# leonsick/s2d

Measured on AMD Instinct MI355X. Metric: clip-frames/sec fwd+loss, R50 M2F-Video T=8 720p Q=100, higher is better.
Workload: dtype f32 (f16x3 MFMA for dense contractions); 1 GPU; KDVideoMaskFormer fwd+loss (student+teacher fwd, GT+KD VideoSetCriterion), c4: 2 clips/GPU x T=8 x 720x1280, Q=100, P=160000, N=10 sparse GT instances/clip, encoder dropout 0.3; clips_per_gpu=2, frames_per_clip=8, parallelism=dp1 (clips sharded, no collective), streams=2

## Files before the change

include/s2d_hip.h:

```cpp
#ifndef S2D_HIP_H
#define S2D_HIP_H
#include <stdint.h>

#ifndef HIP_INCLUDE_HIP_HIP_RUNTIME_API_H
typedef struct ihipStream_t *hipStream_t;
#endif

#ifdef __cplusplus
extern "C" {
#endif

#define S2D_OK 0
#define S2D_ERR_ARG (-1)
#define S2D_ERR_LAUNCH (-2)

int s2d_abi_version(void);

int s2d_set_dense_mode(int mode);


int s2d_gemm_nt_f32(const float *A, const float *B, float *C, int M, int N, int K, long lda, long ldb, long ldc,
                    int batch, long strideA, long strideB, long strideC, const float *scale, const float *bias,
                    const float *res, long ldr, long strideR, int res_rows, int res_cols, int relu, const void *B_split,
                    hipStream_t stream);

int s2d_gemm_nt_dropout_f32(const float *A, const float *B, float *C, int M, int N, int K, long lda, long ldb, long ldc,
                            const float *bias, const float *res, long ldr, int relu, const void *B_split, float p,
                            uint64_t seed, unsigned site, unsigned row0, hipStream_t stream);

int s2d_dropout_f32(const float *x, long M, int N, float p, uint64_t seed, unsigned site, unsigned row0, float *y, hipStream_t stream);

int s2d_gemm_nt_gate_f32(const float *A, const float *B, float *C, int M, int N, int K, long lda, long ldb, long ldc, const float *scale,
                         const float *res, long ldr, const float *gate, long ldg, float gate_scale, const void *B_split, hipStream_t stream);
int s2d_conv2d_nhwc_gate_f32(const float *x, const float *w, float *y, int N, int H, int W, int Cin, int Cout, int KH, int KW, int stride,
                             int pad, const float *scale, const float *gate, float gate_scale, const void *w_split, hipStream_t stream);
int s2d_gemm_nt_presplit_f32(const void *A_split, const float *B, float *C, int M, int N, int K, long ldb, long ldc, const float *bias,
                             const float *res, long ldr, int res_rows, int res_cols, int relu, const void *B_split, hipStream_t stream);
long s2d_split_weights_words(int N, int K);
int s2d_split_weights_f16(const float *W, int N, int K, long ldw, void *out, hipStream_t stream);

long s2d_ffn_pack_words(int C, int F, int Npost, int pre);
int s2d_ffn_pack_f16(const float *W1, const float *W2, int C, int F, const float *Wpost, int Npost, const float *Wpre, void *out,
                     hipStream_t stream);
int s2d_ffn_fused_f32(const float *x, long M, int C, int F, const void *pack, const float *b1, const float *b2, const float *ln1_gamma,
                      const float *ln1_beta, const float *ln2_gamma, const float *ln2_beta, float eps, float p, uint64_t seed,
                      unsigned site_hidden, unsigned site_out, unsigned row0, float *xn, float *y, int Npost, const float *post_bias,
                      const float *post_pos, int post_S, int post_npos, long post_ldpos, float *post_out, long post_ld,
                      const float *pre_bias, const float *pre_res, unsigned site_pre, hipStream_t stream);

int s2d_conv2d_nhwc_f32(const float *x, const float *w, float *y, int N, int H, int W, int Cin, int Cout, int KH,
                        int KW, int stride, int pad, const float *scale, const float *bias, const float *res,
                        int relu, const void *w_split, hipStream_t stream);

int s2d_gemm_nt_amp_f32(const float *A, const float *B, float *C, int M, int N, int K, long lda, long ldb, long ldc, int batch,
                        long strideA, long strideB, long strideC, const float *scale, const float *bias, const float *res, long ldr,
                        long strideR, int res_rows, int res_cols, int relu, hipStream_t stream);
int s2d_conv2d_nhwc_amp_f32(const float *x, const float *w, float *y, int N, int H, int W, int Cin, int Cout, int KH, int KW, int stride,
                            int pad, const float *scale, const float *bias, const float *res, int relu, hipStream_t stream);


int s2d_msda_forward_f32(const float *value, const int64_t *shapes_host, const int64_t *level_start_host,
                         const float *loc, const float *attn_w, int N, int S, int M, int D, int L, int Lq, int P,
                         float *out, hipStream_t stream);

int s2d_msda_backward_f32(const float *value, const int64_t *shapes_host, const int64_t *level_start_host,
                          const float *loc, const float *attn_w, const float *grad_out, int N, int S, int M, int D,
                          int L, int Lq, int P, float *grad_value, float *grad_loc, float *grad_attn_w,
                          hipStream_t stream);

long s2d_msda_backward_workspace_bytes(const int64_t *shapes_host, int N, int M, int L, int Lq, int P);
int s2d_msda_backward_sorted_f32(const float *value, const int64_t *shapes_host, const int64_t *level_start_host,
                                 const float *loc, const float *attn_w, const float *grad_out, int N, int S, int M, int D,
                                 int L, int Lq, int P, float *grad_value, float *grad_loc, float *grad_attn_w, void *workspace,
                                 long workspace_bytes, hipStream_t stream);
int s2d_msda_backward_sorted_strided_f32(const float *value, long ldv, const int64_t *shapes_host, const int64_t *level_start_host,
                                         const float *loc, const float *attn_w, const float *grad_out, int N, int S, int M, int D,
                                         int L, int Lq, int P, float *grad_value, long ldg, float *grad_loc, float *grad_attn_w,
                                         void *workspace, long workspace_bytes, hipStream_t stream);

long s2d_msda_dev_forward_workspace_bytes(void);
int s2d_msda_forward_dev_f32(const float *value, const int64_t *shapes_dev, const int64_t *level_start_dev, const float *loc,
                             const float *attn_w, int N, int S, int M, int D, int L, int Lq, int P, float *out, void *workspace,
                             hipStream_t stream);
long s2d_msda_dev_backward_workspace_bytes(int N, int S, int M, int L, int Lq, int P);
int s2d_msda_backward_dev_f32(const float *value, const int64_t *shapes_dev, const int64_t *level_start_dev, const float *loc,
                              const float *attn_w, const float *grad_out, int N, int S, int M, int D, int L, int Lq, int P,
                              float *grad_value, float *grad_loc, float *grad_attn_w, void *workspace, long workspace_bytes,
                              hipStream_t stream);
int s2d_msda_forward_dev_f64(const double *value, const int64_t *shapes_dev, const int64_t *level_start_dev, const double *loc,
                             const double *attn_w, int N, int S, int M, int D, int L, int Lq, int P, double *out, hipStream_t stream);
int s2d_msda_backward_dev_f64(const double *value, const int64_t *shapes_dev, const int64_t *level_start_dev, const double *loc,
                              const double *attn_w, const double *grad_out, int N, int S, int M, int D, int L, int Lq, int P,
                              double *grad_value, double *grad_loc, double *grad_attn_w, hipStream_t stream);

int s2d_msda_dev_error_word(int *word);
int s2d_msda_dev_status(const void *workspace, int *err_host, hipStream_t stream);

int s2d_msda_fused_forward_f32(const float *value, int ldv, const int64_t *shapes_host, const float *offs_logits, int ldoa,
                               int N, int S, int M, int D, int L, int P, float *out, hipStream_t stream);

int s2d_msda_fused_prep_f32(const float *offs_logits, int ldoa, const int64_t *shapes_host, int N, int S, int M, int L, int P,
                            float *loc, float *attn, hipStream_t stream);
int s2d_msda_fused_chain_f32(const float *attn, const float *grad_loc, const float *grad_attn, const int64_t *shapes_host, int N,
                             int S, int M, int L, int P, float *d_offs_logits, int ldd, hipStream_t stream);
int s2d_msda_fused_backward_query_f32(const float *value, int ldv, const int64_t *shapes_host, const float *offs_logits, int ldoa,
                                      const float *grad_out, int N, int S, int M, int D, int L, int P, float *d_offs_logits, int ldd,
                                      hipStream_t stream);


int s2d_normalize_pad_nhwc4_f32(const uint8_t *frames, int F, int H0, int W0, int Hp, int Wp, const float *mean3_host,
                                const float *std3_host, float *out, hipStream_t stream);

int s2d_maxpool3x3s2_nhwc_f32(const float *x, int N, int H, int W, int C, float *y, hipStream_t stream);
int s2d_maxpool3x3s2_nhwc_idx_f32(const float *x, int N, int H, int W, int C, float *y, unsigned char *argmax, hipStream_t stream);

long s2d_groupnorm_workspace_doubles(int N, int H, int W, int G);
int s2d_groupnorm_nhwc_f32(const float *x, int N, int H, int W, int C, int G, const float *gamma, const float *beta,
                           float eps, const float *up, int hu, int wu, int relu, double *stats_ws, float *y,
                           hipStream_t stream);

int s2d_layernorm_f32(const float *x, const float *res, const float *gamma, const float *beta, long rows, int C,
                      float eps, float *y, hipStream_t stream);

int s2d_add_bcast_f32(const float *x, const float *b, long n, long bn, float *y, hipStream_t stream);

int s2d_pe_sine_f32(int T, int H, int W, int num_pos_feats, const float *add_c, float *out, hipStream_t stream);


int s2d_attn_mask_bits(const float *mask_logits, int ldq, int B, int Q, int T, int hm, int wm, int hl, int wl, int compact,
                       uint32_t *bits, uint32_t *unmasked, hipStream_t stream);

long s2d_attn_workspace_floats(int B, int H, int K);

int s2d_masked_attn_f32(const float *q, const float *k, const float *v, long ldk, long ldv, const uint32_t *bits,
                        const uint32_t *unmasked, int B, int Q, int K, int C, int H, float *workspace, float *out, float *lse,
                        hipStream_t stream);

long s2d_attn_backward_workspace_floats(int B, int H, int K);
int s2d_masked_attn_backward_f32(const float *q, const float *k, const float *v, long ldk, long ldv, const uint32_t *bits,
                                 const uint32_t *unmasked, const float *out, const float *lse, const float *dout, int B, int Q,
                                 int K, int C, int H, float *workspace, float *dq, float *dk, float *dv, hipStream_t stream);
int s2d_masked_attn_backward_strided_f32(const float *q, const float *k, const float *v, long ldk, long ldv, const uint32_t *bits,
                                         const uint32_t *unmasked, const float *out, const float *lse, const float *dout, int B, int Q,
                                         int K, int C, int H, float *workspace, float *dq, float *dk, long lddk, float *dv, long lddv,
                                         hipStream_t stream);


long s2d_matcher_workspace_floats(int NL, int B, int T, int P, int H, int W);

int s2d_matcher_cost_f32(const float *mask_logits, const float *class_logits, const uint8_t *tgt, const int *tgt_count,
                         const float *coords, uint64_t seed, int NL, int B, int Q, int ldq, int T, int hm, int wm, int H,
                         int W, int Nmax, int P, float w_class, float w_mask, float w_dice, float *workspace, float *C,
                         hipStream_t stream);

long s2d_matcher_c_workspace_floats(int NL, int B, int Q, int T, int P, int H, int W);
int s2d_matcher_cost_c_f32(const float *mask_logits, const float *class_logits, int C1, const uint8_t *tgt, const int *tgt_count,
                           const float *coords, uint64_t seed, int NL, int B, int Q, int ldq, int T, int hm, int wm, int H,
                           int W, int Nmax, int P, float w_class, float w_mask, float w_dice, float *workspace, float *C,
                           hipStream_t stream);

int s2d_lsap_f32(const float *C, const int *tgt_count, int nprob, int B, int Q, int Nmax, int *idx_q, int *idx_t,
                 int *n_match, hipStream_t stream);


int s2d_kd_targets_u8(const float *t_class_logits, const float *t_mask_logits, float score_thr, int topk, int B, int Q,
                      int ldq, int T, int hm, int wm, int H, int W, int Nmax, uint8_t *tgt, int *count, int *kept_q,
                      int *nonempty, hipStream_t stream);

long s2d_kd_targets_c_workspace_bytes(int B, int Q, int C1);
int s2d_kd_targets_c_u8(const float *t_class_logits, int C1, const float *t_mask_logits, float score_thr, int topk, int B, int Q,
                        int ldq, int T, int hm, int wm, int H, int W, int Nmax, void *workspace, uint8_t *tgt, int *count, int *kept_q,
                        int *label, int *nonempty, hipStream_t stream);

int s2d_target_nonempty(const uint8_t *tgt, const int *count, int B, int Nmax, int T, int H, int W, int *nonempty,
                        hipStream_t stream);

long s2d_point_loss_workspace_bytes(int NL, int B, int Q, int Nmax, int T, int hm, int wm, int num_points,
                                    float oversample_ratio, float importance_ratio, int H, int W);

int s2d_point_loss_f32(const float *mask_logits, const uint8_t *tgt, const int *tgt_count, const int *nonempty,
                       const int *idx_q, const int *idx_t, const int *n_match, const float *coords_over,
                       const float *coords_rand, uint64_t seed, int NL, int B, int Q, int ldq, int T, int hm, int wm, int H,
                       int W, int Nmax, int num_points, float oversample_ratio, float importance_ratio, int drop_empty,
                       float world_size, void *workspace, float *losses, hipStream_t stream);

int s2d_class_loss_f32(const float *class_logits, const int *idx_q, const int *n_match, int B, int Q, int maxm,
                       float eos_coef, float *loss_ce, hipStream_t stream);

int s2d_class_loss_c_f32(const float *class_logits, int C1, const int *idx_q, const int *n_match, int B, int Q, int maxm,
                         float eos_coef, float *loss_ce, hipStream_t stream);


int s2d_infer_select_f32(const float *class_logits, int Q, int C, int K, float *scores, int *query, int *label,
                         hipStream_t stream);

long s2d_infer_select_c_workspace_bytes(int Q, int C1);
int s2d_infer_select_c_f32(const float *class_logits, int Q, int C1, int K, void *workspace, float *scores, int *query, int *label,
                           hipStream_t stream);

long s2d_infer_workspace_floats(int K, int T, int hm, int wm);

long s2d_mask_bit_words(int T, int oh, int ow);

int s2d_infer_masks_u8(const float *mask_logits, int ldq, int T, int hm, int wm, int Hp, int Wp, int ih, int iw, int oh,
                       int ow, const int *query, int K, float *workspace, uint8_t *masks, uint32_t *bits,
                       hipStream_t stream);

int s2d_pack_mask_bits_u8(const uint8_t *masks, int K, long n, uint32_t *bits, hipStream_t stream);

int s2d_mask_pair_counts_u64(const uint32_t *bits, int K, long words, unsigned long long *inter, hipStream_t stream);


int s2d_rle_count_u8(const uint8_t *masks, int F, int H, int W, int *col_off, int *nbound, int *area, int *bbox,
                     hipStream_t stream);

int s2d_rle_positions_u8(const uint8_t *masks, int F, int H, int W, const int *col_off, const long *frame_off,
                         int *positions, hipStream_t stream);

long s2d_rle_string_workspace_bytes(long ncounts);
int s2d_rle_strings_u8(const int *positions, const long *frame_off, int F, long hw, long ncounts, void *workspace,
                       long workspace_bytes, uint8_t *chars, long *str_off, hipStream_t stream);


int s2d_rle_parse_strings(const uint8_t *chars, const long *str_off, int F, long hw, int *ends, int *nrun, hipStream_t stream);

int s2d_rle_decode_bits(const int *ends, const long *run_off, const int *nrun, int F, int H, int W, uint32_t *bits,
                        hipStream_t stream);

int s2d_mask_plane_areas_u32(const uint32_t *bits, int F, long words_per_plane, unsigned *area, hipStream_t stream);

int s2d_mask_plane_bbox_u32(const uint32_t *bits, int F, int H, int W, long words_per_plane, int *bbox, hipStream_t stream);

int s2d_mask_cross_counts_u64(const uint32_t *a, int D, const uint32_t *b, int G, long words, unsigned long long *inter,
                              hipStream_t stream);

long s2d_mask_boundary_workspace_words(int F, int H, int W, int d);
int s2d_mask_boundary_bits_u32(const uint32_t *bits, int F, int H, int W, int d, uint32_t *workspace, long workspace_words,
                               uint32_t *out, hipStream_t stream);


int s2d_index_planes_u32(const uint8_t *index, int T, int H, int W, int K, uint32_t *planes, uint32_t *void_plane, hipStream_t stream);

int s2d_seg2bmap_bits_u32(const uint32_t *bits, int F, int H, int W, uint32_t *out, hipStream_t stream);

int s2d_disk_dilate_bits_u32(const uint32_t *bits, int F, int H, int W, int R, uint32_t *out, hipStream_t stream);

int s2d_mask_frame_cross_counts_i32(const uint32_t *a, int P, const uint32_t *b, int G, int T, long words_per_frame, int *out,
                                    hipStream_t stream);


long s2d_resize_lds_bytes(int rows_max, int span_q, int kh);

int s2d_resize_bilinear_u8(const uint8_t *src, int T, int H0, int W0, const int *h_bounds, const int *h_coeffs, int kh,
                           const int *v_bounds, const int *v_coeffs, int kv, int H1, int W1, int band_rows, int rows_max,
                           int span_q, uint8_t *dst, hipStream_t stream);


int s2d_gemm_tn_f32(const float *A, const float *B, float *C_slices, int Mo, int No, long rowsA, long rowsB, long lda, long ldb,
                    long chunk, long slice_stride, float *colsum_slices, hipStream_t stream);

int s2d_conv_wgrad_tn_f32(const float *dy, const float *x, int N, int H, int W, int Ci, int Ho, int Wo, int Co, int KH, int KW, int stride,
                          int pad, long chunk, float *part, hipStream_t stream);

int s2d_transpose_f32(const float *in, long R, long C, long ldi, float *out, long ldo, hipStream_t stream);

int s2d_multi_add_f32(const long *table, const int *chunk_tensor, const long *chunk_off, int nchunks, int chunk, hipStream_t stream);

int s2d_reduce_slices_f32(const float *part, int S, long n, long stride, float beta, float *out, hipStream_t stream);
int s2d_reduce_slices_pair_f32(const float *partA, long nA, long strideA, float betaA, float *outA, const float *partB, long nB, long strideB,
                               float betaB, float *outB, int S, hipStream_t stream);

int s2d_colsum_slices_f32(const float *in, long R, long C, long ldi, long rows_per_slice, float *part, hipStream_t stream);

long s2d_layernorm_backward_blocks(long rows);
int s2d_layernorm_backward_f32(const float *x, const float *res, const float *dy, const float *gamma, long rows, int C,
                               float eps, float *dx, float *part, hipStream_t stream);

long s2d_groupnorm_backward_blocks(int N, int H, int W);
int s2d_groupnorm_backward_f32(const float *x, const float *dy, const float *gamma, int N, int H, int W, int C, int G, float eps,
                               double *ws, float *dx, float *part_c, hipStream_t stream);

int s2d_resize_bilinear_backward_nhwc_f32(const float *dy, int N, int H, int W, int C, int hu, int wu, float *dup,
                                          hipStream_t stream);

int s2d_maxpool3x3s2_backward_nhwc_f32(const float *x, const float *dy, int N, int H, int W, int C, float *dx,
                                       hipStream_t stream);
int s2d_maxpool3x3s2_backward_idx_nhwc_f32(const unsigned char *argmax, const float *dy, int N, int H, int W, int C, float *dx,
                                           hipStream_t stream);

int s2d_im2col_nhwc_f32(const float *x, int N, int H, int W, int C, int KH, int KW, int stride, int pad, float *col,
                        hipStream_t stream);

int s2d_pixel_shuffle2_gate_f32(const float *G, int N, int Hg, int Wg, int C, int H, int W, const float *scale, const float *gate, float *dx,
                                hipStream_t stream);

int s2d_relu_scale_backward_f32(const float *dy, const float *y, const float *scale, long n, int C, float *dz, float *dres,
                                hipStream_t stream);

int s2d_relu_gate_add_f32(const float *a, const float *g, const float *y, long n, float *out, hipStream_t stream);


int s2d_optim_grad_norm_f32(const void *const *ptrs, const long *numel, const int *chunk_tensor, const long *chunk_off,
                            int nchunks, int chunk, float inv_scale, float max_norm, double *partial, float *normbuf,
                            hipStream_t stream);

int s2d_optim_adamw_ema_f32(const void *const *ptrs, const long *numel, const double *hyper, const int *chunk_tensor,
                            const long *chunk_off, int nchunks, int chunk, double lr_factor, double beta1, double beta2,
                            double eps, double bias_correction1, double bias_correction2_sqrt, float inv_scale, double ema_m,
                            const float *normbuf, hipStream_t stream);

int s2d_point_loss_backward_f32(const float *mask_logits, const uint8_t *tgt, const int *tgt_count, const int *nonempty,
                                const int *idx_q, const int *idx_t, const int *n_match, const float *coords_over,
                                const float *coords_rand, uint64_t seed, int NL, int B, int Q, int ldq, int T, int hm, int wm,
                                int H, int W, int Nmax, int num_points, float oversample_ratio, float importance_ratio,
                                int drop_empty, float world_size, void *workspace, float w_mask, float w_dice, float *grad_rows,
                                unsigned int *bit_scratch, hipStream_t stream);

int s2d_point_loss_rng_points(uint64_t seed, int hm, int wm, int row0, int nrows, int n_over, float *uv, int *bounds, int *scratch_list,
                              hipStream_t stream);

int s2d_class_loss_backward_f32(const float *class_logits, const int *idx_q, const int *n_match, int B, int Q, int maxm,
                                float eos_coef, float w_ce, float *d_class_logits, hipStream_t stream);

int s2d_class_loss_backward_c_f32(const float *class_logits, int C1, const int *idx_q, const int *n_match, int B, int Q, int maxm,
                                  float eos_coef, float w_ce, float *d_class_logits, hipStream_t stream);


int s2d_tracks_to_masks_u8(const float *tracks, int T, int Np, int H, int W, uint8_t *masks, hipStream_t stream);

int s2d_point_id_counts(const uint8_t *point_masks, const int64_t *idmap, int T, int H, int W, int Hi, int Wi, int max_id,
                        int *counts, int *total, hipStream_t stream);

int s2d_track_point_id_counts(const float *tracks, int T, int P, int H, int W, const int64_t *idmap, int Hi, int Wi, int max_id,
                              int *counts, int *total, hipStream_t stream);

int s2d_idmap_select_masks_u8(const int64_t *idmap, int T, int H, int W, const int *frames, const int *objs, int K, uint8_t *out,
                              hipStream_t stream);

int s2d_idmap_presence_u8(const int64_t *idmap, int T, int Hi, int Wi, int max_id, uint8_t *presence, hipStream_t stream);

long s2d_color_ids_workspace_words(int T);
// ... 69 lines not shown
```

s2d_amd/csrc/gemm_bf16.hip:

```cpp
#include "gemm_epilogue.h"
#include "dropout.h"
#include <stdlib.h>
#include <type_traits>

namespace {

typedef __bf16 bf16x2 __attribute__((ext_vector_type(2)));
typedef __bf16 bf16x8 __attribute__((ext_vector_type(8)));

constexpr int BN = 128, BK = 32, ROWW = 36;

__device__ __forceinline__ void split4_bf16(const f32x4 v, u32x2 &hi, u32x2 &lo)
{
    const f32x2 a = {v[0], v[1]}, b = {v[2], v[3]};
    const bf16x2 ha = __builtin_convertvector(a, bf16x2), hb = __builtin_convertvector(b, bf16x2);
    const unsigned int ua = __builtin_bit_cast(unsigned int, ha), ub = __builtin_bit_cast(unsigned int, hb);
    const f32x2 fa = {__uint_as_float(ua << 16), __uint_as_float(ua & 0xFFFF0000u)};
    const f32x2 fb = {__uint_as_float(ub << 16), __uint_as_float(ub & 0xFFFF0000u)};
    const bf16x2 la = __builtin_convertvector(a - fa, bf16x2), lb = __builtin_convertvector(b - fb, bf16x2);
    hi[0] = ua; hi[1] = ub;
    lo[0] = __builtin_bit_cast(unsigned int, la); lo[1] = __builtin_bit_cast(unsigned int, lb);
}

template <int WM, bool CONV>
// ... 1533 lines not shown
#pragma unroll
            for (int w = 0; w < EV; ++w) {
                if (CONV) v[c][w] *= s.sc[w];
                v[c][w] += s.bi[w];
            }
            if constexpr (DROP) {
                float m[8];
                s2d_dropout8((uint32_t)row + p.drop_row0, (uint32_t)(s.col >> 3), p.drop_stream, p.drop_k0, p.drop_k1, p.drop_thresh, p.drop_scale, m);
                v[c][0][0] *= m[0]; v[c][0][1] *= m[1]; v[c][0][2] *= m[2]; v[c][0][3] *= m[3];
                v[c][EV - 1][0] *= m[4]; v[c][EV - 1][1] *= m[5]; v[c][EV - 1][2] *= m[6]; v[c][EV - 1][3] *= m[7];
            }
#pragma unroll
            for (int w = 0; w < EV; ++w) {
                if (RES) {
#pragma unroll
                    for (int j = 0; j < 4; ++j) v[c][w][j] = __builtin_fmaf(s.rs[c][w][j], s.rmask[w], v[c][w][j]);
                }
#pragma unroll
                for (int j = 0; j < 4; ++j) v[c][w][j] = __builtin_amdgcn_fmed3f(v[c][w][j], relu_lo, __builtin_inff());
            }
            if (cok && row < p.M) {
#pragma unroll
                for (int w = 0; w < EV; ++w)
                    __builtin_amdgcn_raw_buffer_store_b128(__builtin_bit_cast(u32x4, v[c][w]), rsC, (int)s.coff, it * ldc4 + 16 * w, 0);
            }
        }
    };

    f32x4 ra[D][4], rb[D][4];
    unsigned int zm[D];
    EpSet es[D];
    set_tile(0);
#pragma unroll
    for (int d = 0; d < D; ++d) {
        load_set(ra[d], rb[d], zm[d]);
        ep_issue(es[d], false);
        __builtin_amdgcn_sched_barrier(0);
    }
    store_set(ra[0], rb[0], zm[0], 0);
    __builtin_amdgcn_sched_barrier(0);
    load_set(ra[0], rb[0], zm[0]);
    ep_issue(es[0], false);
    __builtin_amdgcn_sched_barrier(0);
    xkt = D; xtile = 0;
    __syncthreads();
    auto body = [&](int q, auto U) {
        constexpr int s = (decltype(U)::value + 1) % D;
        f32x4 ev[CPI][EV];
        ep_read(es[s], ev);
        __builtin_amdgcn_sched_barrier(0);
        store_set(ra[s], rb[s], zm[s], (q + 1) & 1);
        __builtin_amdgcn_sched_barrier(0);
        ep_write(es[s], ev);
        __builtin_amdgcn_sched_barrier(0);
        load_set(ra[s], rb[s], zm[s]);
        ep_issue(es[s], q + D < Q);
        __builtin_amdgcn_sched_barrier(0);
        __syncthreads();
    };
    using U0 = std::integral_constant<int, 0>;
    using U1 = std::integral_constant<int, 1>;
    using U2 = std::integral_constant<int, 2>;
    static_assert(D == 3, "the unrolled bodies below are written for three register sets");
    int q0 = 0;
    for (; q0 + D <= Q; q0 += D) { body(q0, U0{}); body(q0 + 1, U1{}); body(q0 + 2, U2{}); }
    if (q0 < Q) body(q0, U0{});
    if (q0 + 1 < Q) body(q0 + 1, U1{});
    __syncthreads();
    xtile = my_tiles;
    for (int it0 = 0; it0 < EPC; it0 += CPI) {
        xkt = it0 / CPI + 1;
        ep_issue(es[0], true);
        xtile = my_tiles;
        f32x4 ev[CPI][EV];
        ep_read(es[0], ev);
        ep_write(es[0], ev);
    }
}

template <bool CONV>
int launch_f16_hi(const GemmParams &p, int batch, hipStream_t st)
{
    const size_t lds = sizeof(float) * 4 * 64 * 36;
    const int nwg = cdiv(p.M, 128) * cdiv(p.N, 64);
    static int pre = -1;
    if (pre < 0) { const char *e = getenv("S2D_GEMM_HI_PRE"); pre = e ? atoi(e) : 1; }
    if (pre && p.Bsplit && p.res && !p.gate && p.K <= 4 * BK && ((p.N | p.ldc | p.ldr | p.res_cols) & 3) == 0)
        hipLaunchKernelGGL((gemm_f16x3_hi_kernel<CONV, true, true>), dim3(nwg, batch), dim3(256), lds, st, p);
    else if (p.Bsplit) hipLaunchKernelGGL((gemm_f16x3_hi_kernel<CONV, true>), dim3(nwg, batch), dim3(256), lds, st, p);
    else hipLaunchKernelGGL((gemm_f16x3_hi_kernel<CONV, false>), dim3(nwg, batch), dim3(256), lds, st, p);
    S2D_CHECK_LAUNCH();
    return S2D_OK;
}

template <bool CONV, bool PIPE, bool BSPLIT, bool DROP = false>
int launch_f16_v(const GemmParams &p, int batch, hipStream_t st)
{
    const size_t lds = sizeof(unsigned int) * 2 * (128 + BN) * ROWW;
    static S2dDevOnce attr_set;
    if (!attr_set.done()) {
        if (hipFuncSetAttribute(reinterpret_cast<const void *>(gemm_f16x3_kernel<CONV, PIPE, BSPLIT, DROP>),
                                hipFuncAttributeMaxDynamicSharedMemorySize, (int)lds) != hipSuccess)
            return S2D_ERR_LAUNCH;
        attr_set.mark();
    }
    const int nwg = cdiv(p.M, 128) * cdiv(p.N, BN);
    hipLaunchKernelGGL((gemm_f16x3_kernel<CONV, PIPE, BSPLIT, DROP>), dim3(nwg, batch), dim3(256), lds, st, p);
    S2D_CHECK_LAUNCH();
    return S2D_OK;
}

constexpr int WS_CONST_N = 16384;
__global__ void ws_constants_kernel(float *z, float *o)
{
    const int i = blockIdx.x * 256 + threadIdx.x;
    z[i] = 0.f; o[i] = 1.f;
}

int s2d_ws_constants(const float **zeros, const float **ones, hipStream_t st)
{
    static float *buf[16] = {};
    int dev = 0;
    if (hipGetDevice(&dev) != hipSuccess || dev < 0 || dev >= 16) return S2D_ERR_LAUNCH;
    if (!buf[dev]) {
        float *b = nullptr;
        if (hipMalloc(&b, sizeof(float) * 2 * WS_CONST_N) != hipSuccess) return S2D_ERR_LAUNCH;
        hipLaunchKernelGGL(ws_constants_kernel, dim3(WS_CONST_N / 256), dim3(256), 0, st, b, b + WS_CONST_N);
        if (hipStreamSynchronize(st) != hipSuccess) return S2D_ERR_LAUNCH;
        buf[dev] = b;
    }
    *zeros = buf[dev]; *ones = buf[dev] + WS_CONST_N;
    return S2D_OK;
}

template <bool CONV, bool BSPLIT, bool DROP, bool RES, bool ASPLIT = false>
int launch_f16_ws_v(const GemmParams &p, hipStream_t st)
{
    const size_t lds = sizeof(unsigned int) * 2 * (128 + BN) * ROWW + sizeof(float) * 4 * 64 * 68;
    static S2dDevOnce attr_set;
    static int cus = 0;
    if (!attr_set.done()) {
        if (hipFuncSetAttribute(reinterpret_cast<const void *>(gemm_f16x3_ws_kernel<CONV, BSPLIT, DROP, RES, ASPLIT>),
                                hipFuncAttributeMaxDynamicSharedMemorySize, (int)lds) != hipSuccess)
            return S2D_ERR_LAUNCH;
        int dev = 0;
        hipDeviceProp_t prop;
        if (hipGetDevice(&dev) != hipSuccess || hipGetDeviceProperties(&prop, dev) != hipSuccess) return S2D_ERR_LAUNCH;
        cus = prop.multiProcessorCount;
        attr_set.mark();
    }
    const int nwg = cdiv(p.M, 128) * cdiv(p.N, BN);
    GemmParams q = p;
    if (s2d_ws_constants(&q.zeros, &q.ones, st) != S2D_OK) return S2D_ERR_LAUNCH;
    hipLaunchKernelGGL((gemm_f16x3_ws_kernel<CONV, BSPLIT, DROP, RES, ASPLIT>), dim3(nwg < cus ? nwg : cus), dim3(512), lds, st, q);
    S2D_CHECK_LAUNCH();
    return S2D_OK;
}

template <bool CONV, bool BSPLIT, bool DROP>
int launch_f16_ws(const GemmParams &p, hipStream_t st)
{
    return p.res ? launch_f16_ws_v<CONV, BSPLIT, DROP, true>(p, st) : launch_f16_ws_v<CONV, BSPLIT, DROP, false>(p, st);
}

template <bool CONV, bool PIPE>
int launch_f16(const GemmParams &p, int batch, hipStream_t st)
{
    return p.Bsplit ? launch_f16_v<CONV, PIPE, true>(p, batch, st) : launch_f16_v<CONV, PIPE, false>(p, batch, st);
}

int launch_conv7x7s2_stem(const GemmParams &p, hipStream_t st)
{
    static int ph = -1;
    if (ph < 0) { const char *e = getenv("S2D_CONV_STEM_PH"); ph = e ? atoi(e) : 8; }
    const size_t lds16 = sizeof(float) * 4 * 64 * 68, lds8 = sizeof(float) * 4 * 32 * 68;
    static S2dDevOnce attr_set;
    if (!attr_set.done()) {
        if (hipFuncSetAttribute(reinterpret_cast<const void *>(conv7x7s2_c4_halo_kernel<16>), hipFuncAttributeMaxDynamicSharedMemorySize, (int)lds16) != hipSuccess)
            return S2D_ERR_LAUNCH;
        attr_set.mark();
    }
    const int imgs = p.M / (p.Hout * p.Wout);
    if (ph == 16) hipLaunchKernelGGL(conv7x7s2_c4_halo_kernel<16>, dim3(imgs * cdiv(p.Hout, 16) * cdiv(p.Wout, ST_P)), dim3(256), lds16, st, p);
    else hipLaunchKernelGGL(conv7x7s2_c4_halo_kernel<8>, dim3(imgs * cdiv(p.Hout, 8) * cdiv(p.Wout, ST_P)), dim3(256), lds8, st, p);
    S2D_CHECK_LAUNCH();
    return S2D_OK;
}

int launch_conv3x3_halo(const GemmParams &pin, hipStream_t st)
{
    const GemmParams &p = pin;
    int pipe = 0;
    if (const char *e = getenv("S2D_CONV_HALO_PIPE")) pipe = atoi(e);
    const size_t lds = sizeof(float) * 4 * 64 * 68;
    static S2dDevOnce attr_set;
    if (!attr_set.done()) {
        for (const void *fn : {reinterpret_cast<const void *>(conv3x3_f16x3_halo_kernel<8, 2, true>), reinterpret_cast<const void *>(conv3x3_f16x3_halo_kernel<16, 1, true>),
                               reinterpret_cast<const void *>(conv3x3_f16x3_halo_kernel<8, 2, false>), reinterpret_cast<const void *>(conv3x3_f16x3_halo_kernel<16, 1, false>)})
            if (hipFuncSetAttribute(fn, hipFuncAttributeMaxDynamicSharedMemorySize, (int)lds) != hipSuccess) return S2D_ERR_LAUNCH;
        attr_set.mark();
    }
    const int imgs = p.M / (p.Hin * p.Win);
    if (p.N <= 64) {
        const int nwg = imgs * cdiv(p.Hin, 16) * cdiv(p.Win, HT_W);
        if (pipe) hipLaunchKernelGGL((conv3x3_f16x3_halo_kernel<16, 1, true>), dim3(nwg), dim3(256), lds, st, p);
        else hipLaunchKernelGGL((conv3x3_f16x3_halo_kernel<16, 1, false>), dim3(nwg), dim3(256), lds, st, p);
    } else {
        const int nwg = imgs * cdiv(p.Hin, HT_H) * cdiv(p.Win, HT_W) * cdiv(p.N, BN);
        if (pipe) hipLaunchKernelGGL((conv3x3_f16x3_halo_kernel<8, 2, true>), dim3(nwg), dim3(256), lds, st, p);
        else hipLaunchKernelGGL((conv3x3_f16x3_halo_kernel<8, 2, false>), dim3(nwg), dim3(256), lds, st, p);
    }
    S2D_CHECK_LAUNCH();
    return S2D_OK;
}

template <bool CONV, bool BSPLIT>
int launch_w128_v(const GemmParams &p, int batch, hipStream_t st)
{
    const size_t lds = sizeof(float) * 4 * 64 * 68;
    static S2dDevOnce attr_set;
    if (!attr_set.done()) {
        if (hipFuncSetAttribute(reinterpret_cast<const void *>(gemm_bf16x3_w128_kernel<CONV, BSPLIT>),
                                hipFuncAttributeMaxDynamicSharedMemorySize, (int)lds) != hipSuccess)
            return S2D_ERR_LAUNCH;
        attr_set.mark();
    }
    const int nwg = cdiv(p.M, 256) * cdiv(p.N, BN);
    hipLaunchKernelGGL((gemm_bf16x3_w128_kernel<CONV, BSPLIT>), dim3(nwg, batch), dim3(256), lds, st, p);
    S2D_CHECK_LAUNCH();
    return S2D_OK;
}

template <bool CONV>
int launch_w128(const GemmParams &p, int batch, hipStream_t st)
{
    return p.Bsplit ? launch_w128_v<CONV, true>(p, batch, st) : launch_w128_v<CONV, false>(p, batch, st);
}

template <int WM, bool CONV>
int launch_t(const GemmParams &p, int batch, hipStream_t st)
{
    constexpr int BM = 64 * WM;
    const size_t lds = sizeof(unsigned int) * 2 * (BM + BN) * ROWW;
    static S2dDevOnce attr_set;
    if (!attr_set.done()) {
        if (hipFuncSetAttribute(reinterpret_cast<const void *>(gemm_bf16x3_kernel<WM, CONV>),
                                hipFuncAttributeMaxDynamicSharedMemorySize, (int)lds) != hipSuccess)
            return S2D_ERR_LAUNCH;
        attr_set.mark();
    }
    const int nwg = cdiv(p.M, BM) * cdiv(p.N, BN);
    hipLaunchKernelGGL((gemm_bf16x3_kernel<WM, CONV>), dim3(nwg, batch), dim3(128 * WM), lds, st, p);
    S2D_CHECK_LAUNCH();
    return S2D_OK;
}

template <bool BF16>
__global__ __launch_bounds__(256) void split_weights_kernel(const float *__restrict__ W, int N, int K, long ldw, int kblocks,
                                                            unsigned int *__restrict__ out, int vec4)
{
    const long i = (long)blockIdx.x * 256 + threadIdx.x;
    if (i >= (long)N * kblocks * 8) return;
    const int c4 = (int)(i & 7);
    const long nb = i >> 3;
    const int kb = (int)(nb % kblocks);
    const long n = nb / kblocks;
    const int k = kb * 32 + c4 * 4;
    f32x4 v = {0.f, 0.f, 0.f, 0.f};
    if (vec4) { if (k < K) v = *reinterpret_cast<const f32x4 *>(W + n * ldw + k); }
    else {
        float t[4] = {0.f, 0.f, 0.f, 0.f};
#pragma unroll
        for (int j = 0; j < 4; ++j)
            if (k + j < K) t[j] = W[n * ldw + k + j];
#pragma unroll
        for (int j = 0; j < 4; ++j) {
            float r;
            asm volatile("v_mov_b32 %0, %1" : "=v"(r) : "v"(t[j]));
            v[j] = r;
        }
    }
    u32x2 hi, lo;
    if (BF16) split4_bf16(v, hi, lo);
    else split4(v, hi, lo);
    unsigned int *o = out + nb * 32;
    *reinterpret_cast<u32x2 *>(o + c4 * 2) = hi;
    *reinterpret_cast<u32x2 *>(o + 16 + c4 * 2) = lo;
}

}

int s2d_split_weights_launch(const float *W, int N, int K, long ldw, unsigned int *out, hipStream_t st, int bf16)
{
    const int kblocks = (K + 31) / 32;
    const long n = (long)N * kblocks * 8;
    if (n == 0) return S2D_OK;
    const int vec4 = ((K | ldw) & 3) == 0 && (reinterpret_cast<uintptr_t>(W) & 15) == 0;
    if (bf16) hipLaunchKernelGGL(split_weights_kernel<true>, dim3(cdiv(n, 256)), dim3(256), 0, st, W, N, K, ldw, kblocks, out, vec4);
    else hipLaunchKernelGGL(split_weights_kernel<false>, dim3(cdiv(n, 256)), dim3(256), 0, st, W, N, K, ldw, kblocks, out, vec4);
    S2D_CHECK_LAUNCH();
    return S2D_OK;
}

int s2d_launch_gemm_bf16x3(const GemmParams &pin, bool conv, int batch, hipStream_t st, int f16)
{
    GemmParams p = pin;
    const long bA = conv ? (long)(p.M / ((long)p.Hout * p.Wout)) * p.Hin * p.Win * p.Cin * 4L : ((long)(p.M - 1) * p.lda + p.K) * 4L;
    const long bB = ((long)(p.N - 1) * p.ldb + p.K) * 4L;
    if (bA > 0xFFFFFF00L || bB > 0xFFFFFF00L) return S2D_ERR_ARG;
    p.bytesA = (unsigned int)bA; p.bytesB = (unsigned int)bB;
    if (p.Bsplit) {
        if ((batch > 1 && p.sB != 0) || (long)p.N * ((p.K + 31) / 32) * 128L > 0xFFFFFF00L) return S2D_ERR_ARG;
        p.kblocks = (p.K + 31) / 32;
    }
    if (!f16 && (p.Asplit || p.gate || p.drop_thresh)) return S2D_ERR_ARG;
    if (s2d_gemm_small_m_ok(p, conv, batch, f16)) return s2d_launch_gemm_small_m(p, st);
    static int ws = -1;
    if (ws < 0) { const char *e = getenv("S2D_GEMM_WS"); ws = e ? atoi(e) : 0; }

    const long bC = ((long)(p.M - 1) * p.ldc + p.N) * 4L, bR = p.res ? ((long)((p.res_rows ? p.res_rows : p.M) - 1) * p.ldr + p.N) * 4L : 0;
    const bool ws_ok = ws && f16 && batch == 1 && !p.gate && p.N <= WS_CONST_N && (conv || !p.scale) && p.K >= 7 * BK - (BK - 1) && ((p.N | p.ldc | p.ldr | p.res_cols) & 3) == 0 &&
                       (conv ? (p.Cin % 4 == 0 && (p.Bsplit || p.K % BK == 0)) : p.K % BK == 0) &&
                       bC <= 0xFFFFFF00L && bR <= 0xFFFFFF00L && (!p.res_rows || p.res_rows >= 64) &&
                       (!p.drop_thresh || (((p.N | p.ldc) & 7) == 0 && (!p.res || ((p.ldr | p.res_cols) & 7) == 0)));
    if (p.Asplit) {
        const bool ok = f16 && !conv && batch == 1 && p.Bsplit && !p.scale && p.N <= WS_CONST_N && p.K >= 7 * BK - (BK - 1) && p.K % BK == 0 &&
                        ((p.N | p.ldc | p.ldr | p.res_cols) & 3) == 0 && bC <= 0xFFFFFF00L && bR <= 0xFFFFFF00L &&
                        (long)p.M * p.kblocks * 128L <= 0xFFFFFF00L && (!p.res_rows || p.res_rows >= 64) &&
                        (!p.drop_thresh || (((p.N | p.ldc) & 7) == 0 && (!p.res || ((p.ldr | p.res_cols) & 7) == 0)));
        if (!ok) return S2D_ERR_ARG;
        if (p.drop_thresh) return p.res ? launch_f16_ws_v<false, true, true, true, true>(p, st) : launch_f16_ws_v<false, true, true, false, true>(p, st);
        return p.res ? launch_f16_ws_v<false, true, false, true, true>(p, st) : launch_f16_ws_v<false, true, false, false, true>(p, st);
    }
    if (ws_ok && !conv && (ws == 2 || (p.Bsplit && (long)cdiv(p.M, 128) * cdiv(p.N, BN) >= 512))) {
        if (p.drop_thresh) return p.Bsplit ? launch_f16_ws<false, true, true>(p, st) : launch_f16_ws<false, false, true>(p, st);
        return p.Bsplit ? launch_f16_ws<false, true, false>(p, st) : launch_f16_ws<false, false, false>(p, st);
    }
    if (ws_ok && conv && !p.drop_thresh && (ws == 2 || (long)cdiv(p.M, 128) * cdiv(p.N, BN) >= 512)) {
        return p.Bsplit ? launch_f16_ws<true, true, false>(p, st) : launch_f16_ws<true, false, false>(p, st);
    }
    if (p.gate && (!f16 || batch != 1 || p.drop_thresh || ((p.N | p.ldc | p.ldr | p.res_cols | p.ldg) & 3))) return S2D_ERR_ARG;
    if (p.drop_thresh) {
        if (!f16 || conv || ((p.N | p.ldc) & 7) || (p.res && (((p.ldr | p.res_cols) & 7)))) return S2D_ERR_ARG;
        return p.Bsplit ? launch_f16_v<false, true, true, true>(p, batch, st) : launch_f16_v<false, true, false, true>(p, batch, st);
    }
    if (f16) {
        static int halo = -1;
        if (halo < 0) { const char *e = getenv("S2D_CONV_HALO"); halo = e ? atoi(e) : 1; }
        static int stem = -1;
        if (stem < 0) { const char *e = getenv("S2D_CONV_STEM"); stem = e ? atoi(e) : 1; }
        if (stem && conv && p.KH == 7 && p.KW == 7 && p.stride == 2 && p.pad == 3 && p.Cin == 4 && p.N <= 64 && p.N > 32 && p.Bsplit && batch == 1 &&
            ((p.N | p.ldc | p.ldr) & 3) == 0 && !p.res_rows && p.res_cols == p.N && !p.gate && (long)p.Hin * p.Win * 16L * (p.M / ((long)p.Hout * p.Wout)) < 0x7fffffffL)
            return launch_conv7x7s2_stem(p, st);
        static int halo64 = -1;
        if (halo64 < 0) { const char *e = getenv("S2D_CONV_HALO64"); halo64 = e ? atoi(e) : 1; }
        const int ph = p.N <= 64 ? 16 : HT_H;
        if (halo && conv && p.KH == 3 && p.KW == 3 && p.stride == 1 && p.pad == 1 && p.Cin % 32 == 0 && p.Bsplit && batch == 1 && (p.N > 64 || (halo64 && p.N > 32)) &&
            ((p.N | p.ldc | p.ldr) & 3) == 0 && !p.res_rows && p.res_cols == p.N && !p.gate &&
            (halo == 2 || (long)p.Hin * p.Win * 100 >= (long)cdiv(p.Hin, ph) * ph * cdiv(p.Win, HT_W) * HT_W * 88))
            return launch_conv3x3_halo(p, st);
        static int hi = -1;
        if (hi < 0) { const char *e = getenv("S2D_GEMM_HI"); hi = e ? atoi(e) : 2; }
        bool use_hi;
        if (hi != 2) use_hi = hi == 1;
        else if (conv && p.KH > 1) use_hi = p.N <= 64;
        else if (p.N <= 64 || p.K <= 128 || !p.Bsplit) use_hi = true;
        else if (p.K >= 512) use_hi = false;
        else {
            const float w128 = (float)(cdiv(p.N, 128) * 128) / p.N, w64 = (float)(cdiv(p.N, 64) * 64) / p.N;
            use_hi = w128 > w64 + 0.1f;
        }
        if (use_hi) return conv ? launch_f16_hi<true>(p, batch, st) : launch_f16_hi<false>(p, batch, st);
        static int pipe = -1;
        if (pipe < 0) { const char *e = getenv("S2D_GEMM_PIPE"); pipe = e ? atoi(e) : 1; }
        if (pipe) return conv ? launch_f16<true, true>(p, batch, st) : launch_f16<false, true>(p, batch, st);
        return conv ? launch_f16<true, false>(p, batch, st) : launch_f16<false, false>(p, batch, st);
    }
    static int w128 = -1;
    if (w128 < 0) { const char *e = getenv("S2D_GEMM_W128"); w128 = e ? atoi(e) : 1; }
    if (w128 && !conv && (long)cdiv(p.M, 256) * cdiv(p.N, BN) * batch >= (w128 == 2 ? 1 : 512)) return launch_w128<false>(p, batch, st);
    static int force = -1;
    if (force < 0) { const char *e = getenv("S2D_GEMM_WM"); force = e ? atoi(e) : 0; }
    bool big = (long)cdiv(p.M, 256) * cdiv(p.N, BN) * batch >= 256;
    if (force == 2) big = false;
    if (force == 4) big = true;
    if (big) return conv ? launch_t<4, true>(p, batch, st) : launch_t<4, false>(p, batch, st);
    return conv ? launch_t<2, true>(p, batch, st) : launch_t<2, false>(p, batch, st);
}
```

s2d_amd/csrc/gemm_params.h:

```cpp
#pragma once
#include <hip/hip_runtime.h>

struct GemmParams {
    const float *A, *B;
    float *C;
    int M, N, K;
    long lda, ldb, ldc;
    long sA, sB, sC;
    const float *scale, *bias, *res;
    long ldr, sR;
    int res_rows, res_cols;
    int relu;
    const float *gate;
    long ldg;
    float gate_scale;
    int Hin, Win, Cin, Hout, Wout, KH, KW, stride, pad;
    unsigned int bytesA, bytesB;
    const unsigned int *Bsplit;
    int kblocks;
    const unsigned int *Asplit;
    unsigned int drop_thresh;
    float drop_scale;
    unsigned int drop_k0, drop_k1, drop_stream;
    unsigned int drop_row0;
    const float *zeros, *ones;
};


int s2d_split_weights_launch(const float *W, int N, int K, long ldw, unsigned int *out, hipStream_t st, int bf16);
int s2d_launch_gemm_bf16x3(const GemmParams &p, bool conv, int batch, hipStream_t st, int f16);
bool s2d_gemm_small_m_ok(const GemmParams &p, bool conv, int batch, int f16);
int s2d_launch_gemm_small_m(const GemmParams &p, hipStream_t st);
```

Measured before the change: 177.4 clip-frames/s.

## Add row-stationary GEMM kernel for tall small-K f16x3 contractions

Adds a new GEMM path for large-M, small-K (K ≤ 256) problems with pre-split weights. Each 128-row block keeps its A tile split into f16 hi/lo fragments in registers and sweeps every N tile, streaming B through a three-slot LDS ring via buffer loads that write straight to LDS. This avoids reloading and resplitting A for each N tile and cuts launch-grid overhead for tall projections. The path is on by default and selected by a size heuristic. It uses a lot of registers, which may limit occupancy, and it adds a launch counter.

Result: faster. 181.1 clip-frames/s, median of 6 (+2.1%).

```diff
diff --git a/include/s2d_hip.h b/include/s2d_hip.h
--- a/include/s2d_hip.h
+++ b/include/s2d_hip.h
@@ -37,6 +37,7 @@
 int s2d_gemm_nt_presplit_f32(const void *A_split, const float *B, float *C, int M, int N, int K, long ldb, long ldc, const float *bias,
                              const float *res, long ldr, int res_rows, int res_cols, int relu, const void *B_split, hipStream_t stream);
 long s2d_split_weights_words(int N, int K);
+long s2d_gemm_rows_launches(void);
 int s2d_split_weights_f16(const float *W, int N, int K, long ldw, void *out, hipStream_t stream);
 
 long s2d_ffn_pack_words(int C, int F, int Npost, int pre);
diff --git a/s2d_amd/csrc/gemm_bf16.hip b/s2d_amd/csrc/gemm_bf16.hip
--- a/s2d_amd/csrc/gemm_bf16.hip
+++ b/s2d_amd/csrc/gemm_bf16.hip
@@ -1859,6 +1859,12 @@
     return S2D_OK;
 }
 
+static bool gemm_rows_wins(const GemmParams &p)
+{
+    if (p.M >= 65536) return (long)p.N * p.K >= 65536;
+    return p.M >= 32768 && p.N >= 1024 && p.K >= 256;
+}
+
 int s2d_launch_gemm_bf16x3(const GemmParams &pin, bool conv, int batch, hipStream_t st, int f16)
 {
     GemmParams p = pin;
@@ -1871,6 +1877,9 @@
         p.kblocks = (p.K + 31) / 32;
     }
     if (!f16 && (p.Asplit || p.gate || p.drop_thresh)) return S2D_ERR_ARG;
+    int rows = 1;
+    if (const char *e = getenv("S2D_GEMM_ROWS")) rows = atoi(e);
+    if (rows && s2d_gemm_rows_ok(p, conv, batch, f16) && (rows == 2 || gemm_rows_wins(p))) return s2d_launch_gemm_rows(p, st);
     if (s2d_gemm_small_m_ok(p, conv, batch, f16)) return s2d_launch_gemm_small_m(p, st);
     static int ws = -1;
     if (ws < 0) { const char *e = getenv("S2D_GEMM_WS"); ws = e ? atoi(e) : 0; }
diff --git a/s2d_amd/csrc/gemm_params.h b/s2d_amd/csrc/gemm_params.h
--- a/s2d_amd/csrc/gemm_params.h
+++ b/s2d_amd/csrc/gemm_params.h
@@ -31,3 +31,5 @@
 int s2d_launch_gemm_bf16x3(const GemmParams &p, bool conv, int batch, hipStream_t st, int f16);
 bool s2d_gemm_small_m_ok(const GemmParams &p, bool conv, int batch, int f16);
 int s2d_launch_gemm_small_m(const GemmParams &p, hipStream_t st);
+bool s2d_gemm_rows_ok(const GemmParams &p, bool conv, int batch, int f16);
+int s2d_launch_gemm_rows(const GemmParams &p, hipStream_t st);
diff --git a/s2d_amd/csrc/gemm_rows.hip b/s2d_amd/csrc/gemm_rows.hip
--- /dev/null
+++ b/s2d_amd/csrc/gemm_rows.hip
@@ -0,0 +1,228 @@
+#include "gemm_epilogue.h"
+#include <stdlib.h>
+#include <atomic>
+
+bool s2d_gemm_small_m_ok(const GemmParams &p, bool conv, int batch, int f16);
+
+namespace {
+
+constexpr int BM = 128, TN = 64;
+constexpr int GRAN = TN * 128;
+constexpr int STAGE = 2 * GRAN, NSLOT = 3;
+constexpr int EPS = 36;
+constexpr int EPW = 32 * EPS * 4;
+constexpr int LDS_BYTES = NSLOT * STAGE + 4 * EPW;
+
+__device__ __forceinline__ void dma_piece(const u32x4 rs, int voff, int soff, unsigned int dst)
+{
+    unsigned int keep;
+    asm volatile("s_mov_b32 %0, m0\n\ts_mov_b32 m0, %4\n\ts_nop 0\n\tbuffer_load_dwordx4 %1, %2, %3 offen lds\n\ts_mov_b32 m0, %0"
+                 : "=&s"(keep) : "v"(voff), "s"(rs), "s"(soff), "s"(dst) : "memory");
+}
+
+template <int NKB, bool PARTS>
+__global__ __launch_bounds__(256, PARTS ? 1 : 2) void gemm_rows_kernel(GemmParams p)
+{
+    constexpr int SPT = (NKB + 1) / 2;
+    extern __shared__ __attribute__((aligned(16))) unsigned char lds[];
+    const int tid = threadIdx.x, lane = tid & 63;
+    const int wave = __builtin_amdgcn_readfirstlane(tid >> 6);
+    const int l32 = lane & 31, h = lane >> 5;
+    const int m0 = blockIdx.x * BM + wave * 32;
+    const int NT = (p.N + TN - 1) / TN;
+    const int Q = NT * SPT;
+
+    const __amdgpu_buffer_rsrc_t rsA = __builtin_amdgcn_make_buffer_rsrc(const_cast<float *>(p.A), 0, (int)p.bytesA, 0x00020000);
+    const unsigned long long bsp = reinterpret_cast<unsigned long long>(p.Bsplit);
+    const u32x4 rsB = {(unsigned int)bsp, (unsigned int)(bsp >> 32) & 0xFFFFu, (unsigned int)((long)p.N * NKB * 128L), 0x00020000u};
+    const unsigned int lds_base = (unsigned int)reinterpret_cast<uintptr_t>((__attribute__((address_space(3))) unsigned char *)lds);
+
+    auto issue = [&](int t, int sidx, int slot) {
+#pragma unroll
+        for (int e = 0; e < 2; ++e) {
+            const int i = wave * 2 + e;
+            int n = t * TN + i * 8 + (lane >> 3);
+            n = n < p.N ? n : p.N - 1;
+            const int piece = (lane & 7) ^ (e * 4 + (lane >> 4));
+            const int voff = n * (NKB * 128) + piece * 16;
+#pragma unroll
+            for (int g = 0; g < 2; ++g) {
+                const int kb = 2 * sidx + g;
+                if (kb < NKB) dma_piece(rsB, voff, kb * 128, lds_base + slot * STAGE + g * GRAN + i * 1024);
+            }
+        }
+    };
+    issue(0, 0, 0);
+    if (Q > 1) issue(SPT > 1 ? 0 : 1, SPT > 1 ? 1 : 0, 1);
+
+    float *ep = reinterpret_cast<float *>(lds + NSLOT * STAGE + wave * EPW);
+    f16x8 ah[2 * NKB], al[2 * NKB];
+    {
+        const int c8 = lane & 7, r8 = lane >> 3;
+        unsigned int aoff[4];
+#pragma unroll
+        for (int i = 0; i < 4; ++i) {
+            const int m = m0 + i * 8 + r8;
+            aoff[i] = (unsigned int)((long)(m < p.M ? m : p.M - 1) * p.lda * 4L) + (unsigned int)(c8 * 16);
+        }
+        f32x4 ra[2][4];
+#pragma unroll
+        for (int i = 0; i < 4; ++i) ra[0][i] = __builtin_bit_cast(f32x4, __builtin_amdgcn_raw_buffer_load_b128(rsA, (int)aoff[i], 0, 0));
+#pragma unroll
+        for (int kb = 0; kb < NKB; ++kb) {
+            if (kb + 1 < NKB) {
+#pragma unroll
+                for (int i = 0; i < 4; ++i)
+                    ra[(kb + 1) & 1][i] = __builtin_bit_cast(f32x4, __builtin_amdgcn_raw_buffer_load_b128(rsA, (int)aoff[i], (kb + 1) * 128, 0));
+            }
+#pragma unroll
+            for (int i = 0; i < 4; ++i) *reinterpret_cast<f32x4 *>(&ep[(i * 8 + r8) * EPS + c8 * 4]) = ra[kb & 1][i];
+#pragma unroll
+            for (int s = 0; s < 2; ++s) {
+                const f32x4 x0 = *reinterpret_cast<const f32x4 *>(&ep[l32 * EPS + 16 * s + 8 * h]);
+                const f32x4 x1 = *reinterpret_cast<const f32x4 *>(&ep[l32 * EPS + 16 * s + 8 * h + 4]);
+                split8(x0, x1, ah[2 * kb + s], al[2 * kb + s]);
+            }
+        }
+    }
+
+    int boff[4];
+#pragma unroll
+    for (int cc = 0; cc < 4; ++cc) boff[cc] = l32 * 128 + (((2 * cc + h) ^ ((l32 >> 1) & 7)) * 16);
+
+    f32x16 accm[2], accx[2], sum[2];
+#pragma unroll
+    for (int j = 0; j < 2; ++j)
+#pragma unroll
+        for (int r = 0; r < 16; ++r) { accm[j][r] = 0.f; accx[j][r] = 0.f; sum[j][r] = 0.f; }
+
+    if (Q == 1) asm volatile("s_waitcnt vmcnt(0)" ::: "memory");
+    else if ((NKB & 1) && (SPT > 1 ? 1 : 0) == SPT - 1) asm volatile("s_waitcnt vmcnt(2)" ::: "memory");
+    else asm volatile("s_waitcnt vmcnt(4)" ::: "memory");
+
+    const int c4e = lane & 7, rr = lane >> 3;
+    int slot = 0;
+    for (int t = 0; t < NT; ++t) {
+#pragma unroll
+        for (int sidx = 0; sidx < SPT; ++sidx) {
+            asm volatile("s_waitcnt lgkmcnt(0)\n\ts_barrier" ::: "memory");
+            const int s2 = (sidx + 2) % SPT, dt = (sidx + 2) / SPT;
+            const bool more = t + dt < NT;
+            if (more) issue(t + dt, s2, slot >= 1 ? slot - 1 : NSLOT - 1);
+            const unsigned char *sb = lds + slot * STAGE;
+#pragma unroll
+            for (int g = 0; g < 2; ++g) {
+                const int kb = 2 * sidx + g;
+                if (kb >= NKB) continue;
+#pragma unroll
+                for (int s = 0; s < 2; ++s) {
+                    const int ks = 2 * kb + s;
+                    f16x8 bh[2], bl[2];
+#pragma unroll
+                    for (int j = 0; j < 2; ++j) {
+                        bh[j] = *reinterpret_cast<const f16x8 *>(sb + g * GRAN + j * 4096 + boff[s]);
+                        bl[j] = *reinterpret_cast<const f16x8 *>(sb + g * GRAN + j * 4096 + boff[2 + s]);
+                    }
+#pragma unroll
+                    for (int j = 0; j < 2; ++j) {
+                        accx[j] = __builtin_amdgcn_mfma_f32_32x32x16_f16(al[ks], bh[j], accx[j], 0, 0, 0);
+                        accx[j] = __builtin_amdgcn_mfma_f32_32x32x16_f16(ah[ks], bl[j], accx[j], 0, 0, 0);
+                        accm[j] = __builtin_amdgcn_mfma_f32_32x32x16_f16(ah[ks], bh[j], accm[j], 0, 0, 0);
+                    }
+                }
+            }
+            slot = slot + 1 == NSLOT ? 0 : slot + 1;
+            if (!more) { if (t + 1 < NT || sidx + 1 < SPT) asm volatile("s_waitcnt vmcnt(0)" ::: "memory"); }
+            else if ((NKB & 1) && s2 == SPT - 1) asm volatile("s_waitcnt vmcnt(2)" ::: "memory");
+            else asm volatile("s_waitcnt vmcnt(4)" ::: "memory");
+            if constexpr (PARTS) {
+#pragma unroll
+                for (int j = 0; j < 2; ++j)
+#pragma unroll
+                    for (int r = 0; r < 16; ++r) {
+                        sum[j][r] += join(accm[j][r], accx[j][r]);
+                        accm[j][r] = 0.f; accx[j][r] = 0.f;
+                    }
+            }
+        }
+        const int n0 = t * TN;
+#pragma unroll
+        for (int j = 0; j < 2; ++j) {
+            const int col = n0 + j * 32 + c4e * 4;
+            const int colc = col < p.N ? col : p.N - 4;
+            const bool take = col < p.res_cols;
+            f32x4 sc = {1.f, 1.f, 1.f, 1.f}, bi = {0.f, 0.f, 0.f, 0.f}, rs[4];
+            if (p.scale) sc = *reinterpret_cast<const f32x4 *>(p.scale + colc);
+            if (p.bias) bi = *reinterpret_cast<const f32x4 *>(p.bias + colc);
+            if (p.res) {
+                const int colr = take ? col : p.res_cols - 4;
+#pragma unroll
+                for (int it = 0; it < 4; ++it) {
+                    const int row = m0 + it * 8 + rr, rowc = row < p.M ? row : p.M - 1;
+                    rs[it] = *reinterpret_cast<const f32x4 *>(p.res + (long)(p.res_rows ? rowc % p.res_rows : rowc) * p.ldr + colr);
+                }
+            }
+#pragma unroll
+            for (int r = 0; r < 16; ++r) {
+                ep[mfma32_row(r, h) * EPS + l32] = PARTS ? sum[j][r] : join(accm[j][r], accx[j][r]);
+                accm[j][r] = 0.f; accx[j][r] = 0.f; sum[j][r] = 0.f;
+            }
+#pragma unroll
+            for (int it = 0; it < 4; ++it) {
+                const int row = m0 + it * 8 + rr;
+                f32x4 v = *reinterpret_cast<const f32x4 *>(&ep[(it * 8 + rr) * EPS + c4e * 4]);
+                v = v * sc + bi;
+                if (p.res) {
+                    const f32x4 vr = v + rs[it];
+                    v = take ? vr : v;
+                }
+                v = row_act<false>(p, v, row, col);
+                if (row < p.M && col < p.N) *reinterpret_cast<f32x4 *>(p.C + (long)row * p.ldc + col) = v;
+            }
+        }
+    }
+}
+
+std::atomic<long> g_launches{0};
+
+template <int NKB, bool PARTS>
+int launch_rows(const GemmParams &p, hipStream_t st)
+{
+    static S2dDevOnce attr_set;
+    if (!attr_set.done()) {
+        if (hipFuncSetAttribute(reinterpret_cast<const void *>(gemm_rows_kernel<NKB, PARTS>), hipFuncAttributeMaxDynamicSharedMemorySize, LDS_BYTES) != hipSuccess)
+            return S2D_ERR_LAUNCH;
+        attr_set.mark();
+    }
+    hipLaunchKernelGGL((gemm_rows_kernel<NKB, PARTS>), dim3(cdiv(p.M, BM)), dim3(256), LDS_BYTES, st, p);
+    S2D_CHECK_LAUNCH();
+    g_launches.fetch_add(1, std::memory_order_relaxed);
+    return S2D_OK;
+}
+
+}
+
+bool s2d_gemm_rows_ok(const GemmParams &p, bool conv, int batch, int f16)
+{
+    const long bC = ((long)(p.M - 1) * p.ldc + p.N) * 4L, bR = p.res ? ((long)((p.res_rows ? p.res_rows : p.M) - 1) * p.ldr + p.N) * 4L : 0;
+    return f16 && !conv && batch == 1 && p.M >= 1 && p.Bsplit && !p.Asplit && !p.gate && !p.drop_thresh && p.K % 32 == 0 && p.K >= 32 && p.K <= 256 &&
+           p.N >= 128 && ((p.N | p.ldc | p.ldr | p.res_cols) & 3) == 0 && bC <= 0xFFFFFF00L && bR <= 0xFFFFFF00L;
+}
+
+int s2d_launch_gemm_rows(const GemmParams &p, hipStream_t st)
+{
+    const bool parts = s2d_gemm_small_m_ok(p, false, 1, 1) && (p.K == 128 || p.K == 256);
+    switch (p.K / 32) {
+    case 1: return launch_rows<1, false>(p, st);
+    case 2: return launch_rows<2, false>(p, st);
+    case 3: return launch_rows<3, false>(p, st);
+    case 4: return parts ? launch_rows<4, true>(p, st) : launch_rows<4, false>(p, st);
+    case 5: return launch_rows<5, false>(p, st);
+    case 6: return launch_rows<6, false>(p, st);
+    case 7: return launch_rows<7, false>(p, st);
+    case 8: return parts ? launch_rows<8, true>(p, st) : launch_rows<8, false>(p, st);
+    }
+    return S2D_ERR_ARG;
+}
+
+extern "C" long s2d_gemm_rows_launches(void) { return g_launches.load(std::memory_order_relaxed); }
```
